# lyd405121/ti-raytrace

Hardware: AMD Instinct MI355X
Metric: Mrays/s (primary+secondary) at 1024² 100k-tri, 1/2/4/8 GPU + HBM GB/s (higher is better)
Workload: dtype f32

## Files before the change

ti_raytrace_amd/_native.py:

```python
import ctypes as C
import os

import numpy as np

_HERE = os.path.dirname(os.path.abspath(__file__))
LIB_PATH = os.environ.get("TIRT_LIB_PATH") or os.path.join(_HERE, "csrc", "libtirt.so")

_f32p = np.ctypeslib.ndpointer(dtype=np.float32, flags="C_CONTIGUOUS")
_i32p = np.ctypeslib.ndpointer(dtype=np.int32, flags="C_CONTIGUOUS")


class TirtError(RuntimeError):
    pass


class TirtStackOverflow(TirtError):

    def __init__(self, msg, stats):
        TirtError.__init__(self, msg)
        self.stats = stats


ERR_STACK = -4

# ... 32 lines not shown
MOM_MEAN = 1
MOM_M2 = 4
MOM_BAD = 7

MOTION_WORDS = 8

SF_GLASS, SF_ENV, SF_LIGHT_TRI, SF_LIGHT_SPOT_LASER, SF_NO_LIGHT, SF_LIGHT_SPHERE, SF_LIGHT_OTHER = 1, 2, 4, 8, 16, 32, 64
SF_ALL = 127
SF_TEXTURE = 128
SHADE_INSTANTIATIONS = (SF_LIGHT_SPHERE, SF_LIGHT_TRI, SF_ALL, SF_ALL | SF_TEXTURE)
SF_TEXTURE_PARAM = 256
SHADE_INSTANTIATION_MAPS = SF_ALL | SF_TEXTURE | SF_TEXTURE_PARAM
SF_CUTOUT = 512
SF_ENV_SAMPLE = 1024
SHADE_INSTANTIATIONS_ENV = (SF_ALL | SF_ENV_SAMPLE, SHADE_INSTANTIATION_MAPS | SF_ENV_SAMPLE)
KAT_ENV_SAMPLE_IN, KAT_ENV_SAMPLE_OUT = 2, 10
KAT_ENV_PDF_IN, KAT_ENV_PDF_OUT = 3, 5
KAT_ALPHA_IN, KAT_ALPHA_OUT = 3, 2
KAT_MAPS_IN, KAT_MAPS_OUT = 3, 8
KAT_STEP_IN, KAT_STEP_OUT = 23, 28

OPTIONS = {
    "shade_specialize": (1, "1: the narrowest instantiation of k_shade / k_shade_spec that covers the scene's feature word; 0: the generic kernel"),
}

_vp = C.c_void_p
SIGNATURES = {
    "tirt_last_error": (C.c_char_p, []),
    "tirt_version": (C.c_int, []),
    "tirt_device_count": (C.c_int, [C.POINTER(C.c_int)]),
    "tirt_create": (C.c_int, [C.c_int, C.POINTER(_vp)]),
    "tirt_destroy": (None, [_vp]),
    "tirt_sync": (C.c_int, [_vp]),
    "tirt_set_option": (C.c_int, [_vp, C.c_char_p, C.c_double]),
    "tirt_scene_upload": (C.c_int, [_vp, _f32p, C.c_int, _i32p, C.c_int, _f32p, C.c_int,
                                    _f32p, C.c_int, _i32p, C.c_int, C.c_int, _f32p, _f32p]),
    "tirt_material_upload": (C.c_int, [_vp, _f32p, C.c_int]),
    "tirt_env_upload": (C.c_int, [_vp, _i32p, C.c_int, C.c_int, C.c_float]),
    "tirt_texture_upload": (C.c_int, [_vp, C.c_int, _vp, C.c_int64, _vp, _vp, _vp, _vp]),
    "tirt_kat_texture": (C.c_int, [_vp, _f32p, C.c_int, _f32p, C.c_int, C.c_int]),
    "tirt_kat_material_maps": (C.c_int, [_vp, _f32p, C.c_int, _f32p, C.c_int, C.c_int]),
    "tirt_texture_cutout": (C.c_int, [_vp, _vp, C.c_int]),
    "tirt_kat_texture_alpha": (C.c_int, [_vp, _f32p, C.c_int, _f32p, C.c_int, C.c_int]),
    "tirt_shade_features": (C.c_int, [_vp, C.POINTER(C.c_uint32)]),
    "tirt_shade_features_host": (C.c_int, [_f32p, C.c_int, _i32p, C.c_int, _f32p, C.c_int, _i32p, C.c_int, _vp, C.c_int, C.c_int, C.c_float,
                                           C.POINTER(C.c_uint32)]),
# ... 765 lines not shown
```

ti_raytrace_amd/csrc/tirt_api.hip:

```cpp
#include "tirt_internal.h"
#include "tirt_spectral.h"
#include <stddef.h>
#include <algorithm>
#include <mutex>
#include <string.h>

namespace tirt {

static thread_local std::string g_error;
void set_error(const std::string &msg) { g_error = msg; }

SceneView scene_view(const tirt_ctx *c)
{
    SceneView s;
    s.vertex = c->vertex.as<float>(); s.primitive = c->primitive.as<int>(); s.material = c->material.as<float>();
    s.shape = c->shape.as<float>(); s.light = c->light.as<int>(); s.env = c->env.as<int>();
    s.mat_lrgb = c->mat_lrgb.as<float>(); s.shade_rec = c->shade_rec.as<float4>(); s.light_rec = c->light_rec.as<float4>();
    s.tex = c->tex_count > 0 ? c->tex.as<int>() : nullptr;
    s.n = c->n; s.light_count = c->light_count; s.env_w = c->env_w; s.env_h = c->env_h; s.env_power = c->env_power;
    return s;
}
BvhView bvh_view(const tirt_ctx *c)
{
    BvhView b;
// ... 609 lines not shown
    do { if (int rc__ = flush_pending(c)) return rc__; } while (0)

int tirt_sync(tirt_ctx *c)
{
    CTX(c);
    if (sync_all(c)) return TIRT_ERR_HIP;
    TIRT_HIP(hipGetLastError());
    return TIRT_OK;
}

int tirt_set_option(tirt_ctx *c, const char *name, double value)
{
    CTX(c);
    TIRT_REQUIRE(name, "tirt_set_option: null name");
    if (!strcmp(name, "time_kernels")) { c->time_kernels = value != 0.0; return TIRT_OK; }
    if (!strcmp(name, "overlap_lanes")) { TIRT_REQUIRE(value >= 1.0 && value <= (double)TIRT_MAX_LANES, "overlap_lanes: 1..8"); if (sync_all(c)) return TIRT_ERR_HIP; c->n_lanes = (int)value; return TIRT_OK; }
#ifndef TIRT_EXPERIMENTS
    if (!strcmp(name, "wide_collapse")) {
        TIRT_REQUIRE(value == 0.0, "this option is an experiment (cost-optimal wide collapse): build with -DTIRT_EXPERIMENTS (make experiments)");
        return TIRT_OK;
    }
#endif
    if (!strcmp(name, "split_lone_batch")) { TIRT_REQUIRE(value >= 0.0 && value <= 8.0, "split_lone_batch: 0 (off) or the number of parts, 2..8"); c->split_lone = (int)value; return TIRT_OK; }
    if (!strcmp(name, "wide_collapse")) { TIRT_REQUIRE(value == 0.0 || value == 1.0, "wide_collapse: 0 (greedy) or 1 (cost-optimal)"); c->wide_dp_on = (int)value; return TIRT_OK; }
    if (!strcmp(name, "traversal_tree")) {
        TIRT_REQUIRE(value == 0.0 || value == 1.0, "traversal_tree: 0 (the reference's LBVH) or 1 (binned SAH)");
        c->use_sah = (int)value; return TIRT_OK;
    }
    if (!strcmp(name, "plan_batches")) { TIRT_REQUIRE(value >= 0.0 && value <= 64.0, "plan_batches: 0 (automatic) .. 64"); if (flush_pending(c)) return TIRT_ERR_HIP; c->plan_nb = (int)value; return TIRT_OK; }
    if (!strcmp(name, "plan_lanes")) { TIRT_REQUIRE(value >= 0.0 && value <= TIRT_MAX_LANES, "plan_lanes: 0 (automatic) .. the lane count"); if (flush_pending(c)) return TIRT_ERR_HIP; c->plan_lanes = (int)value; return TIRT_OK; }
    if (!strcmp(name, "job_frames")) { TIRT_REQUIRE(value >= 0.0 && value <= 1.0e9, "job_frames out of range"); c->job_frames = (long)value; return TIRT_OK; }
    if (!strcmp(name, "merge_paths")) { TIRT_REQUIRE(value >= 0.0 && value <= 1.0e9, "merge_paths out of range"); c->merge_paths = (size_t)value; c->merge_user = true; return TIRT_OK; }
    if (!strcmp(name, "batch_paths")) {
        TIRT_REQUIRE(value >= 1.0 && value <= 1.0e9, "tirt_set_option: batch_paths out of range");
        c->batch_paths = (size_t)value; c->batch_user = true; return TIRT_OK;
    }
    if (!strcmp(name, "trace_lds_depth")) {
        TIRT_REQUIRE(value >= 12 && value <= 64, "trace_lds_depth: 12..64");
        TIRT_REQUIRE(trace_lds_bytes((int)value) <= c->lds_optin, "trace_lds_depth: stacks + tree top exceed the LDS a block can have on this device");
        c->tr_lds_depth = (int)value; return TIRT_OK;
    }
    if (!strcmp(name, "bdpt_stack_size")) { TIRT_REQUIRE(value >= 16 && value <= 4096, "bdpt_stack_size: 16..4096"); c->bdpt_stack = (int)value; return TIRT_OK; }
    if (!strcmp(name, "trace_timeline")) { c->timeline_arm = (int)value; c->timeline_waves = 0; return TIRT_OK; }
    if (!strcmp(name, "trace_refill_min")) { TIRT_REQUIRE(value >= 1 && value <= 64, "trace_refill_min: 1..64"); c->tr_refill_min = (int)value; return TIRT_OK; }
    if (!strcmp(name, "trace_node_min")) { TIRT_REQUIRE(value >= 1 && value <= 64, "trace_node_min: 1..64"); c->tr_node_min = (int)value; return TIRT_OK; }
    if (!strcmp(name, "bdpt_bounded")) { c->bdpt_bounded = value != 0.0 ? 1 : 0; return TIRT_OK; }
// ... 1011 lines not shown
```

ti_raytrace_amd/csrc/tirt_internal.h:

```cpp
#pragma once
#include <hip/hip_runtime.h>
#include <stdint.h>
#include <stdio.h>
#include <string>
#include <type_traits>
#include <vector>
#include "../../include/tirt.h"
#include "tirt_device.h"

namespace tirt {

void set_error(const std::string &msg);

#define TIRT_HIP(call)                                                                          \
    do {                                                                                        \
        hipError_t e__ = (call);                                                                \
        if (e__ != hipSuccess) {                                                                \
            tirt::set_error(std::string(#call) + ": " + hipGetErrorString(e__));                \
            return TIRT_ERR_HIP;                                                                \
        }                                                                                       \
    } while (0)

#define TIRT_REQUIRE(cond, msg)                                                                 \
    do {                                                                                        \
// ... 142 lines not shown
};

struct TileMap { int tile_rank, tile_count, tile_size, H, blocked, F; const int *pixels; };
TD void slot_to_frame_pixel(const TileMap &m, int P, int slot, int &f, int &k)
{
    if (m.F > 0) { const int c = slot >> 6, kb = c / m.F; f = c - kb * m.F; k = (kb << 6) | (slot & 63); }
    else { f = slot / P; k = slot - f * P; }
}
TD int frame_pixel_to_slot(const TileMap &m, int P, int f, int k)
{ return m.F > 0 ? ((((k >> 6) * m.F + f) << 6) | (k & 63)) : f * P + k; }
TD int local_to_pixel(const TileMap &m, int k)
{
    int lt = k / m.tile_size, within = k - lt * m.tile_size;
    if (m.blocked) {
        const int rows = m.H >> 3;
        const int b = within >> 6, l = within & 63;
        const int bc = b / rows, bj = b - bc * rows;
        within = ((bc << 3) + (l >> 3)) * m.H + (bj << 3) + (l & 7);
    }
    return (lt * m.tile_count + m.tile_rank) * m.tile_size + within;
}

template <bool LIST> TD int mapped_pixel(const TileMap &m, int k) { if constexpr (LIST) return m.pixels[k]; else return local_to_pixel(m, k); }

struct DevCounters {
    unsigned long long rays_closest, rays_shadow, box_closest, leaf_closest, box_shadow, leaf_shadow;
    unsigned long long shaded, paths, stack_overflow;
    unsigned long long it_node, lanes_node, it_leaf, lanes_leaf, refills, it_outer;
    unsigned long long wave_ticks, drain_ticks, waves;
};

#define TIRT_MAX_LANES 8
struct Lane {
    hipStream_t stream = nullptr;
    hipEvent_t film_done = nullptr; bool film_recorded = false;
    hipEvent_t aov_done = nullptr;
    size_t path_capacity = 0;
    DevBuf path_mem, counters_mem, spill;
    PathState ps;
};

}

struct tirt_ctx {
    int device = 0;
    hipStream_t stream = nullptr;
// ... 37 lines not shown

    tirt::CameraView cam; float view[16]; bool cam_set = false;

    int W = 0, H = 0, tile_rank = 0, tile_count = 1, tile_size = 4096, tile_blocked = 0;
    long npix_local = 0;
    tirt::DevBuf hdr, rgb;
    tirt::DevBuf aov;
    hipEvent_t last_aov = nullptr;
    tirt::DevBuf mom, mom_cnt;
    tirt::DevBuf pixset, pixset_tmp; long pixset_n = -1;
    tirt::DevBuf tp_mem; int tp_cur = 0; bool tp_valid = false; tirt_temporal_camera_t tp_cam = {};
    tirt::DevBuf mv_rec, mv_snap; bool mv_moved = false, mv_rec_valid = false;
    tirt::DevBuf dn_mem, dn_out;

    tirt::Lane lanes[TIRT_MAX_LANES];
    int n_lanes = 4;
    unsigned lane_cursor = 0;
    hipEvent_t ev_main = nullptr;
    hipEvent_t last_film = nullptr;
    size_t batch_paths = (size_t)32 << 20;
    size_t merge_paths = (size_t)32 << 20;
    unsigned batches_since_sync = 0;
    int split_lone = 0;
    bool grid_user = false;
    int plan_nb = 0, plan_lanes = 0;
    bool batch_user = false, merge_user = false;
    long job_frames = 0;
    struct { bool valid = false; uint32_t begin = 0; int count = 0; uint32_t seed = 0; int max_depth = 0, stack_size = 0, flags = 0; bool spectral = false; } pend;
    int tr_lds_depth = 16, tr_refill_min = 18, tr_node_min = 38, tr_grid = 1280, tr_slice_log2 = 5, sh_grid = 1024;
    int path_order_blocks = 1, slices_contiguous = 0;
    int tr_grid_alone = 1280;
    tirt::DevBuf counters_mem, spill;
    int cu_count = 256;

    tirt::DevBuf bdpt_px;
    struct BdLane { tirt::DevBuf items, state, rays, hits, qidx, ctr, rad; hipEvent_t delta_done = nullptr, film_done = nullptr; } bd[4];
    int bdpt_lanes = 2;
    int bdpt_state_fill = 0;
    size_t bdpt_batch_items = (size_t)16 << 20;
    size_t bdpt_mem_budget = 0;
    int bdpt_stack = 64;
    int bdpt_bounded = 1;

    struct PvbKey { tirt::CameraView cam; unsigned long long build; int W, H, tile_rank, tile_count, tile_size, tile_blocked, P; } pvb_key;
    bool pvb_valid = false; int primary_beams = 1, primary_beams_min_frames = 16;
    unsigned long long build_serial = 0;
// ... 127 lines not shown
```

ti_raytrace_amd/csrc/tirt_render.hip:

```cpp
#include "tirt_internal.h"
#include "tirt_spectral.h"

namespace tirt {

constexpr int TR_GRID_MAX = 2048;

enum { KIND_CLOSEST = 0, KIND_SHADOW_ACC = 1, KIND_MIXED = 2, KIND_QUERY = 3 };
#if !defined(TIRT_EXPERIMENTS) && (defined(TR_PAD) || defined(TR_PADG))
#error "the bound ladder (TR_PAD / TR_PADG) needs an experiments build: add -DTIRT_EXPERIMENTS"
#endif
struct TraceArgs {
    BvhView bvh;
    const float *ox, *oy, *oz, *dx, *dy, *dz;
    float eye[3];
    const int *count_ptr; int count_fixed;
    float4 *hit;
    const int *sprim, *sdst; const float *sdist, *scr, *scg, *scb; float *rr, *rg, *rb, *fr, *fg, *fb;
    const float *scw; float *rw, *fw;
    int *spill; int spill_depth;
    const float *sox, *soy, *soz, *sdx, *sdy, *sdz; const int *scount_ptr;
    int *fetch; int slice_log2;
    int slices_contig;
    int lds_depth;
    int refill_min;
    int node_min;
    DevCounters *ctr; int2 *per_ray_counts;
    unsigned long long *timeline;
    int no_ray_count;
    const float4 *ray4;
    const int *ray_index;
};
struct TraceArgsCut : TraceArgs { CutView cut; };
template <bool CUTOUT> struct trace_args_of { typedef TraceArgs type; };
template <> struct trace_args_of<true> { typedef TraceArgsCut type; };

struct ShadeStep {
    bool want_next = false, want_shadow = false, shaded = false;
    v3 next_o = V(0.0f, 0.0f, 0.0f), next_d = next_o, next_thr = next_o, sh_o = next_o, sh_d = next_o, sh_c = next_o;
    float next_pdf = 0.0f, sh_dist = 0.0f; int next_spec = 0, sh_expect = -2;
};
template <unsigned FEAT, bool LIST = false>
TD void shade_path(const SceneView &sc, const TileMap &tm, int P, uint32_t frame_begin, uint32_t seed, int bounce, int last_bounce, int slot,
                   const v3 origin, const v3 direction, const float4 hrec, v3 throughout, v3 &radiance, float brdf_pdf, int perfect_spec, ShadeStep &s)
{
    int f, k; slot_to_frame_pixel(tm, P, slot, f, k);
    const uint32_t pixel = (uint32_t)mapped_pixel<LIST>(tm, k);
    const uint32_t frame = frame_begin + (uint32_t)f;
    const uint32_t dim0 = TM_DIM_BOUNCE0 + TM_DIMS_PER_BOUNCE * (uint32_t)bounce;
    const float t = hrec.x;
    constexpr bool ENV_NEE = (FEAT & SF_ENV_SAMPLE) != 0u;
    [[maybe_unused]] float p_env = 0.0f;
    if constexpr (ENV_NEE) p_env = sc.light_count == 0 ? 1.0f : env_table(sc).share;
    if (t < INF_VALUE) {
// ... 223 lines not shown
    } while (0)
#else
#define TR_LADDER_PADS(where) do { } while (0)
#endif

static_assert(std::is_base_of<TraceArgs, TraceArgsCut>::value && sizeof(TraceArgsCut) >= sizeof(TraceArgs) + sizeof(CutView) && sizeof(TraceArgsCut) <= sizeof(TraceArgs) + 2 * sizeof(CutView),
              "TraceArgsCut is TraceArgs with the CutView behind it");
struct CutSource {
    static TD void load(const float4 *&uv, const int *&tex)
    {
        const __attribute__((address_space(4))) TraceArgsCut *ca = (const __attribute__((address_space(4))) TraceArgsCut *)__builtin_amdgcn_kernarg_segment_ptr();
        asm volatile("" : "+s"(ca));
        uv = ca->cut.uv; tex = ca->cut.tex;
    }
};
template <int MODE, bool COUNT, int KIND, bool CUTOUT = false>
__global__ __launch_bounds__(TR_BLOCK, TR_MIN_WAVES) void k_trace(typename trace_args_of<CUTOUT>::type a)
{
    extern __shared__ __attribute__((aligned(16))) int lds_stack[];
    const int TR_LDS_DEPTH = a.lds_depth;
    constexpr bool MAY_SHADOW = (KIND != KIND_CLOSEST);
    constexpr bool STASH = (MODE != TIRT_TRAVERSE_EXHAUSTIVE);
    constexpr bool BOUNDED = MAY_SHADOW && (MODE != TIRT_TRAVERSE_EXHAUSTIVE);
    const int count_c = (KIND == KIND_SHADOW_ACC || KIND == KIND_QUERY) ? 0 : (a.count_ptr ? *a.count_ptr : a.count_fixed);
    const int count_s = (KIND == KIND_CLOSEST) ? 0 : (KIND == KIND_MIXED ? *a.scount_ptr : (a.count_ptr ? *a.count_ptr : a.count_fixed));
    const int count = count_c + count_s;
    const int tid = threadIdx.x, lane = tid & 63;
    const size_t gstride = (size_t)gridDim.x * TR_BLOCK, gtid = (size_t)blockIdx.x * TR_BLOCK + tid;
    const unsigned long long lt_mask = (lane == 0) ? 0ull : (~0ull >> (64 - lane));
    const BvhView &b = a.bvh;

    bool have = false, par = false, is_sh = (KIND == KIND_SHADOW_ACC || KIND == KIND_QUERY);
    int q = 0, cur = TR_SENT, hit_prim = -1, hit_leaf = -1, expect = -3;
    int pend = 0;
    unsigned n_overflow = 0;
    float hit_t = INF_VALUE, hit_u = 0.0f, hit_v = 0.0f, cull_far = 3.0e38f, settle = -1.0f;
    float lim = INF_VALUE;
    unsigned nbox = 0, nleaf = 0;
    RayCtx r = {};
    float gAx = 0.0f, gAy = 0.0f, gAz = 0.0f, gBnx = 0.0f, gBny = 0.0f, gBnz = 0.0f, gBfx = 0.0f, gBfy = 0.0f, gBfz = 0.0f;
    int grotx = 0, groty = 0, grotz = 0;
    bool exhausted = false;
    unsigned long long tk_start = 0, tk_exh = 0;
    if (COUNT) tk_start = wall_clock64();
    const int S_LOG = a.slice_log2, S_MASK = (1 << S_LOG) - 1;
    int home = (int)((blockIdx.x * (TR_BLOCK / 64) + (tid >> 6)) & S_MASK), tried = 0;
    const int full_chunks = count >> 6;
    unsigned long long sum_box = 0, sum_leaf = 0, sum_box_s = 0, sum_leaf_s = 0, n_over = 0;
// ... 47 lines not shown
            const float4 *const c_ray4 = (KIND == KIND_CLOSEST || KIND == KIND_QUERY) ? ca->ray4 : nullptr;
            const int *const c_rindex = (KIND == KIND_QUERY) ? ca->ray_index : nullptr;
            const float c_gm0 = ca->bvh.grid_min[0], c_gm1 = ca->bvh.grid_min[1], c_gm2 = ca->bvh.grid_min[2];
            const float c_ie0 = ca->bvh.inv_extent[0], c_ie1 = ca->bvh.inv_extent[1], c_ie2 = ca->bvh.inv_extent[2];
            const float c_ic0 = ca->bvh.inv_cell[0], c_ic1 = ca->bvh.inv_cell[1], c_ic2 = ca->bvh.inv_cell[2];
            const float c_ce0 = ca->bvh.cell[0], c_ce1 = ca->bvh.cell[1], c_ce2 = ca->bvh.cell[2];
            const float c_rn0 = ca->bvh.root_min[0], c_rn1 = ca->bvh.root_min[1], c_rn2 = ca->bvh.root_min[2];
            const float c_rx0 = ca->bvh.root_max[0], c_rx1 = ca->bvh.root_max[1], c_rx2 = ca->bvh.root_max[2];
            const int c_root = ca->bvh.root_code, c_rootq = ca->bvh.root_qcode, c_farq = ca->bvh.far_qcode;
            asm volatile("" :: "s"(c_fetch), "s"(c_ox), "s"(c_oy), "s"(c_oz), "s"(c_dx), "s"(c_dy), "s"(c_dz), "s"(c_gm0), "s"(c_gm1), "s"(c_gm2), "s"(c_ie0), "s"(c_ie1), "s"(c_ie2),
                         "s"(c_ic0), "s"(c_ic1), "s"(c_ic2), "s"(c_ce0), "s"(c_ce1), "s"(c_ce2), "s"(c_rn0), "s"(c_rn1), "s"(c_rn2), "s"(c_rx0), "s"(c_rx1), "s"(c_rx2));
            if (MAY_SHADOW) asm volatile("" :: "s"(c_sox), "s"(c_soy), "s"(c_soz), "s"(c_sdx), "s"(c_sdy), "s"(c_sdz), "s"(c_sprim), "s"(c_sdist));
            if (KIND == KIND_CLOSEST || KIND == KIND_QUERY) asm volatile("" :: "s"(c_ray4), "s"(c_rindex));
            const unsigned long long fm = idle;
            int my = count;
            if (fm != 0ull && !exhausted) {
            const int n_idle = __popcll(fm);
            if (COUNT) d_refills++;
            const int leader = __ffsll((long long)fm) - 1;
            const bool contig = ca->slices_contig != 0;
            const int Lc__ = ((((count_c + 63) >> 6) + S_MASK) >> S_LOG) << 6, Ls__ = ((((count_s + 63) >> 6) + S_MASK) >> S_LOG) << 6;
            int lenc__ = count_c - home * Lc__; lenc__ = lenc__ < 0 ? 0 : (lenc__ > Lc__ ? Lc__ : lenc__);
            int lens__ = count_s - home * Ls__; lens__ = lens__ < 0 ? 0 : (lens__ > Ls__ ? Ls__ : lens__);
            const int len = contig ? lenc__ + lens__
                                   : (((full_chunks >> S_LOG) + (home < (full_chunks & S_MASK) ? 1 : 0)) << 6) + (home == (full_chunks & S_MASK) ? (count & 63) : 0);
            int base = 0;
            if (lane == leader) base = atomicAdd(c_fetch + home * TR_FETCH_STRIDE, n_idle);
            base = __shfl(base, leader, 64);
            const int v = base + __popcll(fm & lt_mask);
            if (contig) my = v < lenc__ ? home * Lc__ + v : (v < len ? count_c + home * Ls__ + (v - lenc__) : count);
            else my = v < len ? (((((v >> 6) << S_LOG) + home) << 6) | (v & 63)) : count;
            if (base + n_idle >= len) {
                int *const c_drained = c_fetch + TR_SLICES_MAX * TR_FETCH_STRIDE;
                if (lane == leader && base < (len > 0 ? len : 1)) atomicAdd(c_drained, 1);
                if (__hip_atomic_load(c_drained, __ATOMIC_RELAXED, __HIP_MEMORY_SCOPE_AGENT) > S_MASK) tried = S_MASK;
                home = (home + 1) & S_MASK;
                if (++tried > S_MASK) { exhausted = true; if (COUNT) tk_exh = wall_clock64(); }
            }
            }
            const bool setup_now = !have && my < count;
            if (setup_now) {
                q = my;
                if (KIND == KIND_MIXED) { is_sh = my >= count_c; if (is_sh) q = my - count_c; }
                const bool mixed_sh = (KIND == KIND_MIXED) && is_sh;
                v3 o, d; int rec_expect = -3; float rec_bound = -1.0f;
                const bool from_rec = (KIND == KIND_CLOSEST || KIND == KIND_QUERY) && c_ray4 != nullptr;
                if (from_rec) {
                    const size_t ri = (KIND == KIND_QUERY && c_rindex) ? (size_t)c_rindex[q] : (size_t)q;
                    const float4 r0 = c_ray4[2 * ri], r1 = c_ray4[2 * ri + 1];
                    o = V(r0.x, r0.y, r0.z); d = V(r0.w, r1.x, r1.y); rec_expect = __float_as_int(r1.z); rec_bound = r1.w;
                } else {
#define TR_LDS_(p) __builtin_nontemporal_load(&(p))
                    o = mixed_sh ? V(TR_LDS_(c_sox[q]), TR_LDS_(c_soy[q]), TR_LDS_(c_soz[q]))
                                 : ((KIND == KIND_CLOSEST && c_ox == nullptr) ? V(ca->eye[0], ca->eye[1], ca->eye[2]) : V(TR_LDS_(c_ox[q]), TR_LDS_(c_oy[q]), TR_LDS_(c_oz[q])));
                    d = mixed_sh ? V(TR_LDS_(c_sdx[q]), TR_LDS_(c_sdy[q]), TR_LDS_(c_sdz[q])) : V(TR_LDS_(c_dx[q]), TR_LDS_(c_dy[q]), TR_LDS_(c_dz[q]));
                }
                r = make_ray(o, d);
                par = ray_has_parallel_axis(r);
                hit_t = INF_VALUE; hit_u = 0.0f; hit_v = 0.0f; hit_prim = -1; hit_leaf = -1;
                nbox = 1; nleaf = 0; sa = sa_bottom; paged = 0; n_overflow = 0; pend = 0;
                cull_far = 3.0e38f; settle = -1.0f; expect = -3;
                float t_bound = -1.0f;
                if (MAY_SHADOW && is_sh) {
                    expect = from_rec ? rec_expect : TR_LDS_(c_sprim[q]);
                    if (BOUNDED) t_bound = from_rec ? rec_bound : TR_LDS_(c_sdist[q]);
                }
// ... 333 lines not shown
        jx = tm_rand(seed, (uint32_t)p, frame, TM_DIM_JX) - 0.5f;
        jy = tm_rand(seed, (uint32_t)p, frame, TM_DIM_JY) - 0.5f;
    }
    v3 d = camera_ray_direction(cam, i, j, jx, jy);
    __builtin_nontemporal_store(d.x, &ps.dx[s]); __builtin_nontemporal_store(d.y, &ps.dy[s]); __builtin_nontemporal_store(d.z, &ps.dz[s]);
    if (s == 0) atomicAdd(&ctr->paths, (unsigned long long)S);
}

#ifndef SH_BLOCK
#define SH_BLOCK 256
#endif
#ifndef SH_MIN_WAVES
#define SH_MIN_WAVES 5
#endif
#ifndef SH_MIN_WAVES_NARROW
#define SH_MIN_WAVES_NARROW 5
#endif
#ifndef SH_MIN_WAVES_MAPS
#define SH_MIN_WAVES_MAPS 4
#endif
#ifndef SH_MIN_WAVES_ENV
#define SH_MIN_WAVES_ENV 4
#endif
struct ShadeArgs { PathState ps; PathSoA in, out; };
typedef const __attribute__((address_space(4))) ShadeArgs *cold_shade_t;
#define SH_COLD(ca) cold_shade_t ca = (cold_shade_t)__builtin_amdgcn_kernarg_segment_ptr(); asm volatile("" : "+s"(ca))
#define SH_LD(x) __builtin_nontemporal_load(&(x))
#define SH_ST(x, v) __builtin_nontemporal_store((v), &(x))
template <unsigned FEAT, int MIN_WAVES, bool LIST = false>
__global__ __launch_bounds__(SH_BLOCK, MIN_WAVES) void k_shade(ShadeArgs paths_in_kernarg_segment, SceneView sc, TileMap tm, int P,
                                                   uint32_t frame_begin, uint32_t seed, int bounce, int last_bounce,
                                                   const int *count_ptr, int count_fixed, unsigned long long *append_ctr,
                                                   DevCounters *ctr, v3 eye)
{
    __shared__ unsigned s_wcnt[2][SH_BLOCK / 64];
    __shared__ unsigned long long s_base[2];
    const int lane = threadIdx.x & 63, wid = threadIdx.x >> 6;
    const unsigned long long lt_mask = (lane == 0) ? 0ull : (~0ull >> (64 - lane));
    const int count = count_ptr ? *count_ptr : count_fixed;
    const int total = gridDim.x * blockDim.x;
    const int rounds = (count + total - 1) / total;
    unsigned long long n_shaded = 0;
    for (int it = 0; it < rounds; it++) {
        const int q = it * total + blockIdx.x * blockDim.x + threadIdx.x;
        bool live = q < count, want_next = false, want_shadow = false;
        int slot = 0;
        v3 radiance = V(0.0f, 0.0f, 0.0f), next_o = radiance, next_d = radiance, next_thr = radiance;
        v3 sh_o = radiance, sh_d = radiance, sh_c = radiance;
        float next_pdf = 0.0f, sh_dist = 0.0f; int next_spec = 0, sh_expect = -2;
        if (live) {
            const bool first = bounce == 0;
            SH_COLD(ca);
            const int *const c_slot = ca->in.slot; const uint32_t *const c_flags = ca->in.flags; const float4 *const c_hit = ca->ps.hit;
            const float *const c_ox = ca->in.ox, *const c_oy = ca->in.oy, *const c_oz = ca->in.oz, *const c_dx = ca->in.dx, *const c_dy = ca->in.dy, *const c_dz = ca->in.dz;
            const float *const c_tr = ca->in.tr, *const c_tg = ca->in.tg, *const c_tb = ca->in.tb, *const c_rr = ca->in.rr, *const c_rg = ca->in.rg, *const c_rb = ca->in.rb;
            const float *const c_pdf = ca->in.brdf_pdf;
            asm volatile("" :: "s"(c_slot), "s"(c_flags), "s"(c_hit), "s"(c_ox), "s"(c_oy), "s"(c_oz), "s"(c_dx), "s"(c_dy), "s"(c_dz), "s"(c_tr), "s"(c_tg), "s"(c_tb),
                         "s"(c_rr), "s"(c_rg), "s"(c_rb), "s"(c_pdf));
            slot = first ? q : SH_LD(c_slot[q]);
            const v3 origin = first ? eye : V(SH_LD(c_ox[q]), SH_LD(c_oy[q]), SH_LD(c_oz[q]));
            const v3 direction = V(SH_LD(c_dx[q]), SH_LD(c_dy[q]), SH_LD(c_dz[q]));
            typedef float f4nt__ __attribute__((ext_vector_type(4)));
            const f4nt__ hnt__ = __builtin_nontemporal_load((const f4nt__ *)&c_hit[q]);
            const float4 hrec = make_float4(hnt__.x, hnt__.y, hnt__.z, hnt__.w);
            v3 throughout = first ? V(1.0f, 1.0f, 1.0f) : V(SH_LD(c_tr[q]), SH_LD(c_tg[q]), SH_LD(c_tb[q]));
            radiance = first ? V(0.0f, 0.0f, 0.0f) : V(SH_LD(c_rr[q]), SH_LD(c_rg[q]), SH_LD(c_rb[q]));
            float brdf_pdf = first ? 1.0f : SH_LD(c_pdf[q]);
            int perfect_spec = first ? 1 : (int)(SH_LD(c_flags[q]) & 1u);
            ShadeStep ss;
            shade_path<FEAT, LIST>(sc, tm, P, frame_begin, seed, bounce, last_bounce, slot, origin, direction, hrec, throughout, radiance, brdf_pdf, perfect_spec, ss);
            want_next = ss.want_next; want_shadow = ss.want_shadow; if (ss.shaded) n_shaded++;
            next_o = ss.next_o; next_d = ss.next_d; next_thr = ss.next_thr; next_pdf = ss.next_pdf; next_spec = ss.next_spec;
            sh_o = ss.sh_o; sh_d = ss.sh_d; sh_c = ss.sh_c; sh_expect = ss.sh_expect; sh_dist = ss.sh_dist;
        }
        const int par = it & 1;
        const unsigned long long nmask = __ballot(want_next), smask = __ballot(want_shadow);
        if (lane == 0) s_wcnt[par][wid] = (unsigned)__popcll(nmask) | ((unsigned)__popcll(smask) << 16);
        __syncthreads();
        if (threadIdx.x == 0) {
            unsigned tn = 0, tsd = 0;
#pragma unroll
            for (int w = 0; w < SH_BLOCK / 64; w++) { tn += s_wcnt[par][w] & 0xffffu; tsd += s_wcnt[par][w] >> 16; }
            s_base[par] = (tn | tsd) ? atomicAdd(append_ctr, (unsigned long long)tn | ((unsigned long long)tsd << 32)) : 0ull;
        }
        __syncthreads();
        unsigned pn = 0, psd = 0;
#pragma unroll
        for (int w = 0; w < SH_BLOCK / 64; w++) if (w < wid) { pn += s_wcnt[par][w] & 0xffffu; psd += s_wcnt[par][w] >> 16; }
        const unsigned long long bb = s_base[par];
        const int qn = (int)(unsigned)(bb & 0xffffffffull) + (int)pn + __popcll(nmask & lt_mask);
        const int qs = (int)(unsigned)(bb >> 32) + (int)psd + __popcll(smask & lt_mask);
        if (want_next) {
            SH_COLD(ca);
            float *const o_ox = ca->out.ox, *const o_oy = ca->out.oy, *const o_oz = ca->out.oz, *const o_dx = ca->out.dx, *const o_dy = ca->out.dy, *const o_dz = ca->out.dz;
            float *const o_tr = ca->out.tr, *const o_tg = ca->out.tg, *const o_tb = ca->out.tb, *const o_rr = ca->out.rr, *const o_rg = ca->out.rg, *const o_rb = ca->out.rb;
            float *const o_pdf = ca->out.brdf_pdf; uint32_t *const o_flags = ca->out.flags; int *const o_slot = ca->out.slot;
            asm volatile("" :: "s"(o_ox), "s"(o_oy), "s"(o_oz), "s"(o_dx), "s"(o_dy), "s"(o_dz), "s"(o_tr), "s"(o_tg), "s"(o_tb), "s"(o_rr), "s"(o_rg), "s"(o_rb),
                         "s"(o_pdf), "s"(o_flags), "s"(o_slot));
            SH_ST(o_ox[qn], next_o.x); SH_ST(o_oy[qn], next_o.y); SH_ST(o_oz[qn], next_o.z);
            SH_ST(o_dx[qn], next_d.x); SH_ST(o_dy[qn], next_d.y); SH_ST(o_dz[qn], next_d.z);
            SH_ST(o_tr[qn], next_thr.x); SH_ST(o_tg[qn], next_thr.y); SH_ST(o_tb[qn], next_thr.z);
            SH_ST(o_rr[qn], radiance.x); SH_ST(o_rg[qn], radiance.y); SH_ST(o_rb[qn], radiance.z);
            SH_ST(o_pdf[qn], next_pdf); SH_ST(o_flags[qn], (uint32_t)next_spec); SH_ST(o_slot[qn], slot);
        } else if (live) {
            SH_COLD(ca);
            float *const f_r = ca->ps.fr, *const f_g = ca->ps.fg, *const f_b = ca->ps.fb;
// ... 330 lines not shown
    din.release(); dout.release();
    return rc;
}

__global__ void k_film_spec(PathState ps, const float *fw, SpecView sp, TileMap tm, int P, int F, uint32_t frame_begin, uint32_t seed, float *hdr)
{
    int k = blockIdx.x * blockDim.x + threadIdx.x;
    if (k >= P) return;
    const int p = local_to_pixel(tm, k);
    float *px = hdr + (size_t)p * 3;
    float r = px[0], g = px[1], b = px[2];
    for (int f = 0; f < F; f++) {
        const int s = frame_pixel_to_slot(tm, P, f, k);
        const uint32_t frame = frame_begin + (uint32_t)f;
        const float coff = 1.0f / ((float)(int)frame + 1.0f);
        const float Lambda = HERO_LAMBDA_MIN + HERO_LAMBDA_STEP * tm_rand(seed, (uint32_t)p, frame, TM_DIM_SPEC_LAMBDA);
        f4s spec; spec.v[0] = ps.fr[s]; spec.v[1] = ps.fg[s]; spec.v[2] = ps.fb[s]; spec.v[3] = fw[s];
        spec_add_splat(sp, spec, Lambda, coff, r, g, b);
    }
    px[0] = r; px[1] = g; px[2] = b;
}

constexpr size_t LINE = 128;
static size_t lane_counter_bytes(int max_depth)
{ return LINE * (size_t)(max_depth + 1) + sizeof(int) * TR_FETCH_STRIDE * TR_FETCH_LINES * (size_t)(max_depth + 1); }

constexpr int PATH_WORDS = 2 * 15 + 4 + 12 + 3 + 2;
static size_t path_state_bytes(size_t S) { return sizeof(float) * PATH_WORDS * ((S + 3) & ~(size_t)3); }
static int ensure_paths(Lane &L, size_t S, int max_depth)
{
    if (S > L.path_capacity || !L.path_mem.p) {
        if (L.path_mem.ensure(path_state_bytes(S))) return TIRT_ERR_HIP;
        const size_t S_user = S;
        S = (S + 3) & ~(size_t)3;
        float *w = L.path_mem.as<float>();
        PathState &p = L.ps;
        auto nxt = [&]() { float *r = w; w += S; return r; };
        for (int k = 0; k < 2; k++) {
            PathSoA &q = p.st[k];
            q.ox = nxt(); q.oy = nxt(); q.oz = nxt(); q.dx = nxt(); q.dy = nxt(); q.dz = nxt();
            q.tr = nxt(); q.tg = nxt(); q.tb = nxt(); q.rr = nxt(); q.rg = nxt(); q.rb = nxt();
            q.brdf_pdf = nxt(); q.flags = (uint32_t *)nxt(); q.slot = (int *)nxt();
        }
        p.hit = (float4 *)w; w += 4 * S;
        p.sox = nxt(); p.soy = nxt(); p.soz = nxt(); p.sdx = nxt(); p.sdy = nxt(); p.sdz = nxt();
        p.scr = nxt(); p.scg = nxt(); p.scb = nxt(); p.sprim = (int *)nxt(); p.sdist = nxt(); p.sdst = (int *)nxt();
        p.fr = nxt(); p.fg = nxt(); p.fb = nxt();
        p.scw = nxt(); p.fw = nxt();
// ... 46 lines not shown
    }
    for (int k = 0; k < n_lanes; k++) {
        if (k > 0 && cap > c->lanes[k].path_capacity) {
            size_t free_b = 0, total_b = 0;
            if (hipMemGetInfo(&free_b, &total_b) == hipSuccess && free_b < path_state_bytes(cap) + ((size_t)2 << 30)) { n_lanes = k; break; }
        }
        if (ensure_paths(c->lanes[k], cap, max_depth)) return TIRT_ERR_HIP;
        if (ensure_spill(c, c->lanes[k].spill, stack_size, spill_depth)) return TIRT_ERR_HIP;
    }

    for (int fb = 0; fb < frame_count; fb += FB) {
        Lane &L = c->lanes[n_lanes == 1 ? 0 : (c->lane_cursor++ % (unsigned)n_lanes)];
        c->batches_since_sync++;
        hipStream_t st = L.stream;
        const int F = (frame_count - fb < FB) ? frame_count - fb : FB;
        const int S = F * P;
        tm.F = (c->path_order_blocks && (P & 63) == 0) ? F : 0;
        const bool use_beams = beams_ready && F >= c->primary_beams_min_frames;
        const uint32_t f0 = frame_begin + (uint32_t)fb;
        char *cm = L.counters_mem.as<char>();
        auto append_ctr = [&](int b) { return (unsigned long long *)(cm + LINE * (size_t)b); };
        auto cnt_path = [&](int b) { return (const int *)append_ctr(b - 1); };
        auto cnt_shadow = [&](int b) { return (const int *)append_ctr(b) + 1; };
        auto fetch = [&](int launch) { return (int *)(cm + LINE * (size_t)(max_depth + 1)) + (size_t)launch * TR_FETCH_STRIDE * TR_FETCH_LINES; };

        TIRT_HIP(hipStreamWaitEvent(st, c->ev_main, 0));
        hipEvent_t r0, r1;
        TIRT_HIP(hipEventCreate(&r0)); TIRT_HIP(hipEventCreate(&r1));
        TIRT_HIP(hipEventRecord(r0, st));
        std::vector<std::pair<hipEvent_t, hipEvent_t>> evc, evs, evh;
        auto stamp = [&](std::vector<std::pair<hipEvent_t, hipEvent_t>> &v, bool begin) {
            if (!c->time_kernels) return;
            if (begin) { hipEvent_t a, b; (void)hipEventCreate(&a); (void)hipEventCreate(&b); v.push_back({a, b}); (void)hipEventRecord(a, st); }
            else (void)hipEventRecord(v.back().second, st);
        };

        TIRT_HIP(hipMemsetAsync(L.counters_mem.p, 0, lane_counter_bytes(max_depth), st));
        hipLaunchKernelGGL(list ? k_generate<true> : k_generate<false>, dim3((S + B - 1) / B), dim3(B), 0, st, L.ps.st[0], c->cam, tm, P, S, f0, seed, ctr);
        bool busy = false;
        if (c->last_film) { busy = hipEventQuery(c->last_film) == hipErrorNotReady; (void)hipGetLastError(); }
        const BatchPlan plan = plan_batches(c);
        const bool two_big = plan.lanes <= 2 && plan.batch >= ((size_t)24 << 20) && !c->grid_user;
        const int grid_cap = (busy && n_lanes > 1 && !two_big) ? c->tr_grid : c->tr_grid_alone;
        int grid_full = (S + TR_BLOCK - 1) / TR_BLOCK; if (grid_full > grid_cap) grid_full = grid_cap;
        const int sh_cap = two_big ? 2 * c->sh_grid : c->sh_grid;
        int grid_shade = (S + SH_BLOCK - 1) / SH_BLOCK; if (grid_shade > sh_cap) grid_shade = sh_cap;
        v3 eye_v; eye_v.x = c->cam.eye[0]; eye_v.y = c->cam.eye[1]; eye_v.z = c->cam.eye[2];
        const shade_fn_t shade_fn = list ? pick_shade_rgb(c).fn_list : pick_shade_rgb(c).fn;
        const shade_spec_fn_t shade_spec_fn = pick_shade_inst(SHADE_SPEC_INST, c).fn;
        for (int b = 0; b < max_depth; b++) {
            const PathSoA &in = L.ps.st[b & 1], &out = L.ps.st[(b + 1) & 1];
            TraceArgs a = {};
            a.bvh = bv;
            a.ox = in.ox; a.oy = in.oy; a.oz = in.oz; a.dx = in.dx; a.dy = in.dy; a.dz = in.dz;
            if (b == 0) { a.ox = a.oy = a.oz = nullptr; for (int k = 0; k < 3; k++) a.eye[k] = c->cam.eye[k]; }
            a.count_ptr = (b == 0) ? nullptr : cnt_path(b); a.count_fixed = S;
            a.hit = L.ps.hit;
            a.spill = L.spill.as<int>(); a.spill_depth = spill_depth; a.ctr = ctr; a.per_ray_counts = nullptr;
            a.fetch = fetch(b);
            a.sox = L.ps.sox; a.soy = L.ps.soy; a.soz = L.ps.soz; a.sdx = L.ps.sdx; a.sdy = L.ps.sdy; a.sdz = L.ps.sdz;
            a.sprim = L.ps.sprim; a.sdst = L.ps.sdst; a.sdist = L.ps.sdist; a.scr = L.ps.scr; a.scg = L.ps.scg; a.scb = L.ps.scb;
            a.rr = in.rr; a.rg = in.rg; a.rb = in.rb; a.fr = L.ps.fr; a.fg = L.ps.fg; a.fb = L.ps.fb;
            if (spec) { a.scw = L.ps.scw; a.rw = (float *)in.flags; a.fw = L.ps.fw; }
            a.scount_ptr = (b == 0) ? nullptr : cnt_shadow(b - 1);
            fill_tunables(c, a);
            a.timeline = timeline_for(c, flags, grid_full);
            if (!(b == 0 && use_beams)) stamp(evc, true);
            if (b == 0 && use_beams) {
                int *const fb_count = (int *)append_ctr(0) + 4;
                float4 *const fb_hit = (float4 *)L.ps.sox;
                pvb_launch_cand(c, st, bv, in.dx, in.dy, in.dz, tm, P, S, L.ps.hit, fb_count, (int *)out.ox, out.dx, out.dy, out.dz, ctr);
                TraceArgs a2 = a;
                a2.dx = out.dx; a2.dy = out.dy; a2.dz = out.dz; a2.count_ptr = fb_count; a2.count_fixed = S; a2.hit = fb_hit; a2.no_ray_count = 1;
                stamp(evc, true);
                if (int rc = launch_trace<KIND_CLOSEST>(c, st, a2, flags, grid_full)) return rc;
                stamp(evc, false);
                pvb_launch_scatter(st, fb_count, (const int *)out.ox, fb_hit, L.ps.hit);
            } else
            if (int rc = (b == 0) ? launch_trace<KIND_CLOSEST>(c, st, a, flags, grid_full) : launch_trace<KIND_MIXED>(c, st, a, flags, grid_full)) return rc;
            if (!(b == 0 && use_beams)) stamp(evc, false);
            c->launches_trace_closest++;
            if (b == 0 && c->aov.p) { if (int rc = aov_launch(c, L, tm, P, F, f0)) return rc; }

            stamp(evh, true);
            if (spec)
                hipLaunchKernelGGL(shade_spec_fn, dim3(grid_shade), dim3(SH_BLOCK), 0, st, ShadeArgs{L.ps, in, out}, sv, *spec, tm, P, f0, seed, b,
                                   (b == max_depth - 1) ? 1 : 0, (b == 0) ? (const int *)nullptr : cnt_path(b), S,
                                   append_ctr(b), ctr, eye_v);
            else
            hipLaunchKernelGGL(shade_fn, dim3(grid_shade), dim3(SH_BLOCK), 0, st, ShadeArgs{L.ps, in, out}, sv, tm, P, f0, seed, b,
                               (b == max_depth - 1) ? 1 : 0, (b == 0) ? (const int *)nullptr : cnt_path(b), S,
                               append_ctr(b), ctr, eye_v);
            stamp(evh, false);
            c->launches_shade++;

            if (b == max_depth - 1) {
                TraceArgs sa = {};
                sa.bvh = bv;
                sa.ox = L.ps.sox; sa.oy = L.ps.soy; sa.oz = L.ps.soz; sa.dx = L.ps.sdx; sa.dy = L.ps.sdy; sa.dz = L.ps.sdz;
                sa.count_ptr = cnt_shadow(b); sa.count_fixed = 0;
                sa.sprim = L.ps.sprim; sa.sdst = L.ps.sdst; sa.sdist = L.ps.sdist; sa.scr = L.ps.scr; sa.scg = L.ps.scg; sa.scb = L.ps.scb;
                sa.rr = out.rr; sa.rg = out.rg; sa.rb = out.rb; sa.fr = L.ps.fr; sa.fg = L.ps.fg; sa.fb = L.ps.fb;
                if (spec) { sa.scw = L.ps.scw; sa.rw = (float *)out.flags; sa.fw = L.ps.fw; }
                sa.spill = L.spill.as<int>(); sa.spill_depth = spill_depth; sa.ctr = ctr; sa.per_ray_counts = nullptr;
                sa.fetch = fetch(max_depth);
                fill_tunables(c, sa);
                stamp(evs, true);
                if (int rc = launch_trace<KIND_SHADOW_ACC>(c, st, sa, flags, grid_full)) return rc;
                stamp(evs, false);
                c->launches_trace_shadow++;
            }
        }
        if (c->last_film) TIRT_HIP(hipStreamWaitEvent(st, c->last_film, 0));
        if (spec) hipLaunchKernelGGL(k_film_spec, dim3((P + B - 1) / B), dim3(B), 0, st, L.ps, L.ps.fw, *spec, tm, P, F, f0, seed, c->hdr.as<float>());
        else hipLaunchKernelGGL(list ? k_film<true> : k_film<false>, dim3((P + B - 1) / B), dim3(B), 0, st, L.ps, tm, P, F, f0, c->hdr.as<float>());
        if (c->mom.p && !spec) { if (int rc = moments_launch(c, L, tm, P, F)) return rc; }
        TIRT_HIP(hipEventRecord(L.film_done, st));
        L.film_recorded = true;
        c->last_film = L.film_done;
        if (use_beams) c->pvb_set[c->pvb_cur].busy = L.film_done;
        TIRT_HIP(hipEventRecord(r1, st));
        if (c->time_kernels) {
            TIRT_HIP(hipStreamSynchronize(st));
// ... 26 lines not shown
```

Before: 5657.

## Split shade append counter into two ends of path and shadow queues

```diff
diff --git a/ti_raytrace_amd/_native.py b/ti_raytrace_amd/_native.py
--- a/ti_raytrace_amd/_native.py
+++ b/ti_raytrace_amd/_native.py
@@ -78,6 +78,7 @@
 
 OPTIONS = {
     "shade_specialize": (1, "1: the narrowest instantiation of k_shade / k_shade_spec that covers the scene's feature word; 0: the generic kernel"),
+    "shade_append_ends": (2, "2: k_shade (PT_RGB) appends to both ends of the path and shadow-ray queues through two counters; 1: one counter, dense queues"),
 }
 
 _vp = C.c_void_p
diff --git a/ti_raytrace_amd/csrc/tirt_api.hip b/ti_raytrace_amd/csrc/tirt_api.hip
--- a/ti_raytrace_amd/csrc/tirt_api.hip
+++ b/ti_raytrace_amd/csrc/tirt_api.hip
@@ -655,6 +655,7 @@
     }
 #endif
     if (!strcmp(name, "split_lone_batch")) { TIRT_REQUIRE(value >= 0.0 && value <= 8.0, "split_lone_batch: 0 (off) or the number of parts, 2..8"); c->split_lone = (int)value; return TIRT_OK; }
+    if (!strcmp(name, "shade_append_ends")) { TIRT_REQUIRE(value == 1.0 || value == 2.0, "shade_append_ends: 1 (one append counter) or 2 (both ends of the queues)"); if (flush_pending(c)) return TIRT_ERR_HIP; c->shade_append_ends = (int)value; return TIRT_OK; }
     if (!strcmp(name, "wide_collapse")) { TIRT_REQUIRE(value == 0.0 || value == 1.0, "wide_collapse: 0 (greedy) or 1 (cost-optimal)"); c->wide_dp_on = (int)value; return TIRT_OK; }
     if (!strcmp(name, "traversal_tree")) {
         TIRT_REQUIRE(value == 0.0 || value == 1.0, "traversal_tree: 0 (the reference's LBVH) or 1 (binned SAH)");
diff --git a/ti_raytrace_amd/csrc/tirt_internal.h b/ti_raytrace_amd/csrc/tirt_internal.h
--- a/ti_raytrace_amd/csrc/tirt_internal.h
+++ b/ti_raytrace_amd/csrc/tirt_internal.h
@@ -188,6 +188,8 @@
 }
 
 template <bool LIST> TD int mapped_pixel(const TileMap &m, int k) { if constexpr (LIST) return m.pixels[k]; else return local_to_pixel(m, k); }
+
+TD int phys(int i, int nA, int nB, int cap) { return i < nA ? i : cap - (nA + nB) + i; }
 
 struct DevCounters {
     unsigned long long rays_closest, rays_shadow, box_closest, leaf_closest, box_shadow, leaf_shadow;
@@ -271,6 +273,7 @@
     size_t merge_paths = (size_t)32 << 20;
     unsigned batches_since_sync = 0;
     int split_lone = 0;
+    int shade_append_ends = 2;
     bool grid_user = false;
     int plan_nb = 0, plan_lanes = 0;
     bool batch_user = false, merge_user = false;
diff --git a/ti_raytrace_amd/csrc/tirt_render.hip b/ti_raytrace_amd/csrc/tirt_render.hip
--- a/ti_raytrace_amd/csrc/tirt_render.hip
+++ b/ti_raytrace_amd/csrc/tirt_render.hip
@@ -29,6 +29,7 @@
     int no_ray_count;
     const float4 *ray4;
     const int *ray_index;
+    const int *count_ptr2, *scount_ptr2; int cap, scap;
 };
 struct TraceArgsCut : TraceArgs { CutView cut; };
 template <bool CUTOUT> struct trace_args_of { typedef TraceArgs type; };
@@ -298,8 +299,10 @@
     constexpr bool MAY_SHADOW = (KIND != KIND_CLOSEST);
     constexpr bool STASH = (MODE != TIRT_TRAVERSE_EXHAUSTIVE);
     constexpr bool BOUNDED = MAY_SHADOW && (MODE != TIRT_TRAVERSE_EXHAUSTIVE);
-    const int count_c = (KIND == KIND_SHADOW_ACC || KIND == KIND_QUERY) ? 0 : (a.count_ptr ? *a.count_ptr : a.count_fixed);
-    const int count_s = (KIND == KIND_CLOSEST) ? 0 : (KIND == KIND_MIXED ? *a.scount_ptr : (a.count_ptr ? *a.count_ptr : a.count_fixed));
+    constexpr bool TWO_ENDS = (KIND == KIND_MIXED || KIND == KIND_SHADOW_ACC);
+    const int n_first = a.count_ptr ? *a.count_ptr + ((TWO_ENDS && a.count_ptr2) ? *a.count_ptr2 : 0) : a.count_fixed;
+    const int count_c = (KIND == KIND_SHADOW_ACC || KIND == KIND_QUERY) ? 0 : n_first;
+    const int count_s = (KIND == KIND_CLOSEST) ? 0 : (KIND == KIND_MIXED ? *a.scount_ptr + (a.scount_ptr2 ? *a.scount_ptr2 : 0) : n_first);
     const int count = count_c + count_s;
     const int tid = threadIdx.x, lane = tid & 63;
     const size_t gstride = (size_t)gridDim.x * TR_BLOCK, gtid = (size_t)blockIdx.x * TR_BLOCK + tid;
@@ -393,8 +396,10 @@
             const int Lc__ = ((((count_c + 63) >> 6) + S_MASK) >> S_LOG) << 6, Ls__ = ((((count_s + 63) >> 6) + S_MASK) >> S_LOG) << 6;
             int lenc__ = count_c - home * Lc__; lenc__ = lenc__ < 0 ? 0 : (lenc__ > Lc__ ? Lc__ : lenc__);
             int lens__ = count_s - home * Ls__; lens__ = lens__ < 0 ? 0 : (lens__ > Ls__ ? Ls__ : lens__);
+            int count_r = count; if (TWO_ENDS) asm volatile("" : "+s"(count_r));
+            const int chunks_r = TWO_ENDS ? count_r >> 6 : full_chunks;
             const int len = contig ? lenc__ + lens__
-                                   : (((full_chunks >> S_LOG) + (home < (full_chunks & S_MASK) ? 1 : 0)) << 6) + (home == (full_chunks & S_MASK) ? (count & 63) : 0);
+                                   : (((chunks_r >> S_LOG) + (home < (chunks_r & S_MASK) ? 1 : 0)) << 6) + (home == (chunks_r & S_MASK) ? (count_r & 63) : 0);
             int base = 0;
             if (lane == leader) base = atomicAdd(c_fetch + home * TR_FETCH_STRIDE, n_idle);
             base = __shfl(base, leader, 64);
@@ -413,6 +418,16 @@
             if (setup_now) {
                 q = my;
                 if (KIND == KIND_MIXED) { is_sh = my >= count_c; if (is_sh) q = my - count_c; }
+                typedef const __attribute__((address_space(4))) int *const_int_t;
+                const_int_t c_cnt = TWO_ENDS ? (const_int_t)ca->count_ptr : nullptr, c_cnt2 = TWO_ENDS ? (const_int_t)ca->count_ptr2 : nullptr;
+                const_int_t c_scnt = (KIND == KIND_MIXED) ? (const_int_t)ca->scount_ptr : nullptr, c_scnt2 = (KIND == KIND_MIXED) ? (const_int_t)ca->scount_ptr2 : nullptr;
+                const int c_cap = TWO_ENDS ? ca->cap : 0, c_scap = (KIND == KIND_MIXED) ? ca->scap : 0;
+                if (TWO_ENDS) asm volatile("" : "+s"(c_cnt), "+s"(c_cnt2), "+s"(c_scnt), "+s"(c_scnt2) : "s"(c_cap), "s"(c_scap));
+                const int n_c = (KIND == KIND_MIXED) ? count_c : count_s;
+                int lo_c = n_c, lo_s = count_s;
+                if (TWO_ENDS && c_cnt2) lo_c = *c_cnt;
+                if (KIND == KIND_MIXED && c_scnt2) lo_s = *c_scnt;
+                if (TWO_ENDS) q = (KIND == KIND_MIXED && is_sh) ? phys(q, lo_s, count_s - lo_s, c_scap) : phys(q, lo_c, n_c - lo_c, c_cap);
                 const bool mixed_sh = (KIND == KIND_MIXED) && is_sh;
                 v3 o, d; int rec_expect = -3; float rec_bound = -1.0f;
                 const bool from_rec = (KIND == KIND_CLOSEST || KIND == KIND_QUERY) && c_ray4 != nullptr;
@@ -792,7 +807,12 @@
 #ifndef SH_MIN_WAVES_ENV
 #define SH_MIN_WAVES_ENV 4
 #endif
-struct ShadeArgs { PathState ps; PathSoA in, out; };
+struct ShadeArgs {
+    PathState ps; PathSoA in, out;
+    unsigned long long *append_hi;
+    const int *count_lo, *count_hi;
+    int cap;
+};
 typedef const __attribute__((address_space(4))) ShadeArgs *cold_shade_t;
 #define SH_COLD(ca) cold_shade_t ca = (cold_shade_t)__builtin_amdgcn_kernarg_segment_ptr(); asm volatile("" : "+s"(ca))
 #define SH_LD(x) __builtin_nontemporal_load(&(x))
@@ -807,13 +827,13 @@
     __shared__ unsigned long long s_base[2];
     const int lane = threadIdx.x & 63, wid = threadIdx.x >> 6;
     const unsigned long long lt_mask = (lane == 0) ? 0ull : (~0ull >> (64 - lane));
-    const int count = count_ptr ? *count_ptr : count_fixed;
+    const int count = (count_ptr ? *count_ptr : count_fixed) + (paths_in_kernarg_segment.count_hi ? *paths_in_kernarg_segment.count_hi : 0);
     const int total = gridDim.x * blockDim.x;
     const int rounds = (count + total - 1) / total;
     unsigned long long n_shaded = 0;
     for (int it = 0; it < rounds; it++) {
-        const int q = it * total + blockIdx.x * blockDim.x + threadIdx.x;
-        bool live = q < count, want_next = false, want_shadow = false;
+        const int ql = it * total + blockIdx.x * blockDim.x + threadIdx.x;
+        bool live = ql < count, want_next = false, want_shadow = false;
         int slot = 0;
         v3 radiance = V(0.0f, 0.0f, 0.0f), next_o = radiance, next_d = radiance, next_thr = radiance;
         v3 sh_o = radiance, sh_d = radiance, sh_c = radiance;
@@ -825,9 +845,13 @@
             const float *const c_ox = ca->in.ox, *const c_oy = ca->in.oy, *const c_oz = ca->in.oz, *const c_dx = ca->in.dx, *const c_dy = ca->in.dy, *const c_dz = ca->in.dz;
             const float *const c_tr = ca->in.tr, *const c_tg = ca->in.tg, *const c_tb = ca->in.tb, *const c_rr = ca->in.rr, *const c_rg = ca->in.rg, *const c_rb = ca->in.rb;
             const float *const c_pdf = ca->in.brdf_pdf;
+            typedef const __attribute__((address_space(4))) int *const_int_t;
+            const_int_t c_lo = (const_int_t)ca->count_lo, c_up = (const_int_t)ca->count_hi; const int c_cap = ca->cap;
             asm volatile("" :: "s"(c_slot), "s"(c_flags), "s"(c_hit), "s"(c_ox), "s"(c_oy), "s"(c_oz), "s"(c_dx), "s"(c_dy), "s"(c_dz), "s"(c_tr), "s"(c_tg), "s"(c_tb),
-                         "s"(c_rr), "s"(c_rg), "s"(c_rb), "s"(c_pdf));
-            slot = first ? q : SH_LD(c_slot[q]);
+                         "s"(c_rr), "s"(c_rg), "s"(c_rb), "s"(c_pdf), "s"(c_lo), "s"(c_up), "s"(c_cap));
+            const int n_lo = c_up ? *c_lo : count;
+            const int q = phys(ql, n_lo, count - n_lo, c_cap);
+            slot = first ? ql : SH_LD(c_slot[q]);
             const v3 origin = first ? eye : V(SH_LD(c_ox[q]), SH_LD(c_oy[q]), SH_LD(c_oz[q]));
             const v3 direction = V(SH_LD(c_dx[q]), SH_LD(c_dy[q]), SH_LD(c_dz[q]));
             typedef float f4nt__ __attribute__((ext_vector_type(4)));
@@ -851,7 +875,17 @@
             unsigned tn = 0, tsd = 0;
 #pragma unroll
             for (int w = 0; w < SH_BLOCK / 64; w++) { tn += s_wcnt[par][w] & 0xffffu; tsd += s_wcnt[par][w] >> 16; }
-            s_base[par] = (tn | tsd) ? atomicAdd(append_ctr, (unsigned long long)tn | ((unsigned long long)tsd << 32)) : 0ull;
+            unsigned long long first = 0ull;
+            if (tn | tsd) {
+                const unsigned long long add = (unsigned long long)tn | ((unsigned long long)tsd << 32);
+                SH_COLD(ca);
+                unsigned long long *const c_hi = ca->append_hi; const unsigned c_cap = (unsigned)ca->cap;
+                asm volatile("" :: "s"(c_hi), "s"(c_cap));
+                const bool down = c_hi != nullptr && (blockIdx.x & 1u);
+                first = atomicAdd(down ? c_hi : append_ctr, add);
+                if (down) first = (unsigned long long)(c_cap - (unsigned)(first & 0xffffffffull) - tn) | ((unsigned long long)(c_cap - (unsigned)(first >> 32) - tsd) << 32);
+            }
+            s_base[par] = first;
         }
         __syncthreads();
         unsigned pn = 0, psd = 0;
@@ -1228,8 +1262,9 @@
 }
 
 constexpr size_t LINE = 128;
+static size_t lane_fetch_bytes(int max_depth) { return sizeof(int) * TR_FETCH_STRIDE * TR_FETCH_LINES * (size_t)(max_depth + 1); }
 static size_t lane_counter_bytes(int max_depth)
-{ return LINE * (size_t)(max_depth + 1) + sizeof(int) * TR_FETCH_STRIDE * TR_FETCH_LINES * (size_t)(max_depth + 1); }
+{ return LINE * (size_t)(max_depth + 1) + lane_fetch_bytes(max_depth) + LINE * (size_t)(max_depth + 1); }
 
 constexpr int PATH_WORDS = 2 * 15 + 4 + 12 + 3 + 2;
 static size_t path_state_bytes(size_t S) { return sizeof(float) * PATH_WORDS * ((S + 3) & ~(size_t)3); }
@@ -1322,6 +1357,11 @@
         auto append_ctr = [&](int b) { return (unsigned long long *)(cm + LINE * (size_t)b); };
         auto cnt_path = [&](int b) { return (const int *)append_ctr(b - 1); };
         auto cnt_shadow = [&](int b) { return (const int *)append_ctr(b) + 1; };
+        const bool two_ends = c->shade_append_ends >= 2 && !spec;
+        char *const cm_hi = cm + LINE * (size_t)(max_depth + 1) + lane_fetch_bytes(max_depth);
+        auto append_hi = [&](int b) { return two_ends ? (unsigned long long *)(cm_hi + LINE * (size_t)b) : (unsigned long long *)nullptr; };
+        auto cnt_path_hi = [&](int b) { return (const int *)append_hi(b - 1); };
+        auto cnt_shadow_hi = [&](int b) { return two_ends ? (const int *)append_hi(b) + 1 : (const int *)nullptr; };
         auto fetch = [&](int launch) { return (int *)(cm + LINE * (size_t)(max_depth + 1)) + (size_t)launch * TR_FETCH_STRIDE * TR_FETCH_LINES; };
 
         TIRT_HIP(hipStreamWaitEvent(st, c->ev_main, 0));
@@ -1363,6 +1403,7 @@
             a.rr = in.rr; a.rg = in.rg; a.rb = in.rb; a.fr = L.ps.fr; a.fg = L.ps.fg; a.fb = L.ps.fb;
             if (spec) { a.scw = L.ps.scw; a.rw = (float *)in.flags; a.fw = L.ps.fw; }
             a.scount_ptr = (b == 0) ? nullptr : cnt_shadow(b - 1);
+            if (b > 0) { a.count_ptr2 = cnt_path_hi(b); a.scount_ptr2 = cnt_shadow_hi(b - 1); a.cap = a.scap = S; }
             fill_tunables(c, a);
             a.timeline = timeline_for(c, flags, grid_full);
             if (!(b == 0 && use_beams)) stamp(evc, true);
@@ -1384,11 +1425,11 @@
 
             stamp(evh, true);
             if (spec)
-                hipLaunchKernelGGL(shade_spec_fn, dim3(grid_shade), dim3(SH_BLOCK), 0, st, ShadeArgs{L.ps, in, out}, sv, *spec, tm, P, f0, seed, b,
+                hipLaunchKernelGGL(shade_spec_fn, dim3(grid_shade), dim3(SH_BLOCK), 0, st, ShadeArgs{L.ps, in, out, nullptr, nullptr, nullptr, 0}, sv, *spec, tm, P, f0, seed, b,
                                    (b == max_depth - 1) ? 1 : 0, (b == 0) ? (const int *)nullptr : cnt_path(b), S,
                                    append_ctr(b), ctr, eye_v);
             else
-            hipLaunchKernelGGL(shade_fn, dim3(grid_shade), dim3(SH_BLOCK), 0, st, ShadeArgs{L.ps, in, out}, sv, tm, P, f0, seed, b,
+            hipLaunchKernelGGL(shade_fn, dim3(grid_shade), dim3(SH_BLOCK), 0, st, ShadeArgs{L.ps, in, out, append_hi(b), (b == 0) ? (const int *)nullptr : cnt_path(b), (b == 0) ? (const int *)nullptr : cnt_path_hi(b), S}, sv, tm, P, f0, seed, b,
                                (b == max_depth - 1) ? 1 : 0, (b == 0) ? (const int *)nullptr : cnt_path(b), S,
                                append_ctr(b), ctr, eye_v);
             stamp(evh, false);
@@ -1398,7 +1439,7 @@
                 TraceArgs sa = {};
                 sa.bvh = bv;
                 sa.ox = L.ps.sox; sa.oy = L.ps.soy; sa.oz = L.ps.soz; sa.dx = L.ps.sdx; sa.dy = L.ps.sdy; sa.dz = L.ps.sdz;
-                sa.count_ptr = cnt_shadow(b); sa.count_fixed = 0;
+                sa.count_ptr = cnt_shadow(b); sa.count_fixed = 0; sa.count_ptr2 = cnt_shadow_hi(b); sa.cap = S;
                 sa.sprim = L.ps.sprim; sa.sdst = L.ps.sdst; sa.sdist = L.ps.sdist; sa.scr = L.ps.scr; sa.scg = L.ps.scg; sa.scb = L.ps.scb;
                 sa.rr = out.rr; sa.rg = out.rg; sa.rb = out.rb; sa.fr = L.ps.fr; sa.fg = L.ps.fg; sa.fb = L.ps.fb;
                 if (spec) { sa.scw = L.ps.scw; sa.rw = (float *)out.flags; sa.fw = L.ps.fw; }
```

After: 5665 (median of 3 runs). Within noise of the previous version (+0.1%).
